# compbio-UofT/shrimp

Measured on AMD Instinct MI355X. Metric: reads/sec mapped (whole node), 100bp LS reads vs 3Gbp ref, 1/2/4/8 GPUs, higher is better.
Workload: dtype int16

## Files before the change

include/gmapper_hip.h:

```cpp
#ifndef GMAPPER_HIP_H
#define GMAPPER_HIP_H

#include <stddef.h>
#include <stdint.h>
#include <stdbool.h>

#ifdef __cplusplus
extern "C" {
#endif

#define GM_OK            0
#define GM_E_NODEVICE   -1
#define GM_E_ARG        -2
#define GM_E_NOTSETUP   -3
#define GM_E_RANGE      -4
#define GM_E_OVERFLOW   -5
#define GM_E_NOMEM      -6

const char *gm_last_error(void);
int gm_abi_sizeof(int which);
int gm_device_count(void);

typedef struct gm_params {
  int match_score, mismatch_score;
// ... 233 lines not shown
  int half_paired;
  int match_mode;
} gm_pair_opts_t;
void gm_pair_opts_default(gm_pair_opts_t *o);
int gm_map_pairs(gm_session_t *s, int n_pairs, int len1, const uint32_t *mates1_packed, int len2, const uint32_t *mates2_packed,
                 const char *names1, const char *names2, const gm_pair_opts_t *opts,
                 char **sam, size_t *sam_len, gm_map_stats_t *stats);
int gm_map_pairs_cs(gm_session_t *s, int n_pairs, int len1, const uint32_t *mates1_packed, const uint8_t *initbp1, int len2, const uint32_t *mates2_packed,
                    const uint8_t *initbp2, const char *names1, const char *names2, const gm_pair_opts_t *opts,
                    char **sam, size_t *sam_len, gm_map_stats_t *stats);
int gm_map_pairs_file(gm_session_t *s, const char *path1, const char *path2, int fastq, int qual_delta, const gm_pair_opts_t *opts,
                      char **sam, size_t *sam_len, gm_map_stats_t *stats);
int gm_map_pairs_file_cb(gm_session_t *s, const char *path1, const char *path2, int fastq, int qual_delta, const gm_pair_opts_t *opts, size_t chunk_pairs,
                         gm_write_fn write, void *ctx, gm_map_stats_t *stats);
int gm_map_pairs_cs_fastq(gm_session_t *s, int n_pairs, int len1, const uint32_t *mates1_packed, const uint8_t *initbp1, int len2, const uint32_t *mates2_packed,
                          const uint8_t *initbp2, const char *names1, const char *names2, const char *quals1, const char *quals2, int qual_delta,
                          const gm_pair_opts_t *opts, char **sam, size_t *sam_len, gm_map_stats_t *stats);
int gm_map_pairs_fastq(gm_session_t *s, int n_pairs, int len1, const uint32_t *mates1_packed, int len2, const uint32_t *mates2_packed,
                       const char *names1, const char *names2, const char *quals1, const char *quals2, int qual_delta,
                       const gm_pair_opts_t *opts, char **sam, size_t *sam_len, gm_map_stats_t *stats);

#define GM_MERGE_OUT_SAM              0
#define GM_MERGE_OUT_UNALIGNED_READS  1
#define GM_MERGE_OUT_ALIGNED_READS    2
typedef struct gm_merge_options {
  int max_outputs;
  int max_alignments;
  int strata;
  int half_paired;
  int sam_unaligned;
  int single_best;
  int all_contigs;
  int no_mapping_qualities;
  int leave_mapq;
  int no_improper_mappings;
  int min_mapq;
  int fastq;
  int threads;
  int output;
  int header_given;
  const char *command_line;
} gm_merge_options_t;
void gm_merge_options_default(gm_merge_options_t *o);
int gm_merge_sam(const gm_merge_options_t *opts, const char *reads_text, size_t reads_len, int n_files, const char *const *sam_text,
                 const size_t *sam_len, char **out, size_t *out_len);

int gm_debug_tophits(gm_session_t *s, int n_reads, int read_len, const uint32_t *reads_packed,
                     long long *rows, long cap, long *n_rows);
int gm_debug_tophits_cs(gm_session_t *s, int n_reads, int n_colours, const uint32_t *colours_packed, const uint8_t *initbp,
                        long long *rows, long cap, long *n_rows);

int gm_last_lookup_timing(gm_session_t *s, double *ms, uint64_t *alg_bytes, int *launches);
const char *gm_last_lookup_kernel(void);

#ifdef __cplusplus
}
#endif
#endif
```

shrimp_amd/csrc/gm_anchors.hip:

```cpp
#include <cstring>
#include <algorithm>
#include "gm_common.h"
#include "gm_internal.h"
#include <rocprim/device/device_segmented_radix_sort.hpp>

template <bool BIG> struct K2Idx { typedef uint16_t type; static constexpr uint32_t none = 0xFFFFu; };
template <> struct K2Idx<true> { typedef uint32_t type; static constexpr uint32_t none = 0xFFFFFFFFu; };

template <bool BIG>
struct K2Ws {
  typedef typename K2Idx<BIG>::type idx_t;
  uint64_t* key;
  uint32_t* aux;
  idx_t* nxt;
  idx_t* ord;
  idx_t* first;
  uint32_t* hk;
  uint16_t* hr;
  int16_t*  cache;
};

#ifdef K2_STAMPS
__device__ unsigned long long k2_stamps[8];
#define K2_STAMP(i) do { if (lane == 0) { const unsigned long long t_ = __builtin_amdgcn_s_memtime(); atomicAdd(&k2_stamps[i], t_ - t_prev); t_prev = t_; } } while (0)
extern "C" int gm_debug_k2_stamps(unsigned long long* out) {
  unsigned long long z[8] = {0, 0, 0, 0, 0, 0, 0, 0};
  if (hipMemcpyFromSymbol(out, HIP_SYMBOL(k2_stamps), sizeof z) != hipSuccess) return GM_E_NODEVICE;
  if (hipMemcpyToSymbol(HIP_SYMBOL(k2_stamps), z, sizeof z) != hipSuccess) return GM_E_NODEVICE;
  return GM_OK;
}
#else
#define K2_STAMP(i) do { } while (0)
#endif
template <bool BIG> __device__ __forceinline__ void k2_sync() { if (BIG) __threadfence(); __syncthreads(); }

template <bool BIG, typename T> __device__ void k2_bitonic(T* key, int npad, int lane) {
  for (int k = 2; k <= npad; k <<= 1)
    for (int j = k >> 1; j > 0; j >>= 1) {
      for (int t = lane; t < (npad >> 1); t += GM_WAVE) {
        const int i = ((t & ~(j - 1)) << 1) | (t & (j - 1));
        const int l = i | j;
        const bool up = ((i & k) == 0);
        const T a = key[i], b = key[l];
        if ((a > b) == up) { key[i] = b; key[l] = a; }
      }
      k2_sync<BIG>();
    }
}

template <typename T> __device__ __forceinline__ T k2_xor_lane(T v, int dl) { return (T)__shfl_xor(v, dl); }
template <> __device__ __forceinline__ uint64_t k2_xor_lane<uint64_t>(uint64_t v, int dl) {
  const uint32_t lo = (uint32_t)__shfl_xor((int)(uint32_t)v, dl), hi = (uint32_t)__shfl_xor((int)(uint32_t)(v >> 32), dl);
  return ((uint64_t)hi << 32) | lo;
}
template <typename T, int R> __device__ __forceinline__ void k2_bitonic_regs(T* key, int lane) {
  T v[R];
#pragma unroll
  for (int j = 0; j < R; j++) v[j] = key[lane * R + j];
#pragma unroll
  for (int k = 2; k <= 64 * R; k <<= 1) {
#pragma unroll
    for (int d = k >> 1; d > 0; d >>= 1) {
      if (d < R) {
#pragma unroll
        for (int j = 0; j < R; j++) if ((j & d) == 0) {
          const bool up = (((lane * R + j) & k) == 0);
          const T a = v[j], b = v[j | d];
          const bool sw = (a > b) == up;
          v[j] = sw ? b : a; v[j | d] = sw ? a : b;
        }
      } else {
        const int dl = d / R;
        const bool lower = (lane & dl) == 0;
#pragma unroll
        for (int j = 0; j < R; j++) {
          const bool up = (((lane * R + j) & k) == 0);
          const T o = k2_xor_lane<T>(v[j], dl);
          const bool less = v[j] < o;
          v[j] = ((up == lower) == less) ? v[j] : o;
        }
      }
    }
  }
#pragma unroll
  for (int j = 0; j < R; j++) key[lane * R + j] = v[j];
}
template <bool BIG, typename T, int RMAX = 16> __device__ void k2_sort(T* key, int npad, int lane) {
  if (!BIG && npad <= 64 * RMAX) {
    if (npad == 64) k2_bitonic_regs<T, 1>(key, lane); else if (npad == 128) k2_bitonic_regs<T, 2>(key, lane);
    else if (npad == 256) k2_bitonic_regs<T, 4>(key, lane); else if (npad == 512) k2_bitonic_regs<T, 8>(key, lane);
    else if (npad == 1024 || RMAX < 32) k2_bitonic_regs<T, 16>(key, lane);
    else k2_bitonic_regs<T, RMAX>(key, lane);
    __syncthreads();
  } else k2_bitonic<BIG, T>(key, npad, lane);
}

struct K2Box { long long x, y; int length, width; };
__device__ __forceinline__ K2Box k2_join2(long long x0, long long y0, int l0, int w0, long long x1, long long y1, int l1, int w1) {
  long long nw0 = x0 + y0, sw0 = x0 - y0, ne0 = sw0 + 2 * (w0 - 1), se0 = nw0 + 2 * (l0 - 1);
  long long nw1 = x1 + y1, sw1 = x1 - y1, ne1 = sw1 + 2 * (w1 - 1), se1 = nw1 + 2 * (l1 - 1);
  long long nw_min = min(nw0, nw1), sw_min = min(sw0, sw1), ne_max = max(ne0, ne1), se_max = max(se0, se1);
  K2Box r;
  if ((nw_min + sw_min) % 2 != 0) nw_min--;
  r.x = (nw_min + sw_min) / 2;
  r.y = nw_min - r.x;
  if ((ne_max - sw_min) % 2 != 0) ne_max++;
  r.width = (int)((ne_max - sw_min) / 2 + 1);
  if ((se_max - nw_min) % 2 != 0) se_max++;
  r.length = (int)((se_max - nw_min) / 2 + 1);
  return r;
}

__device__ __forceinline__ int k2_threshold(double frac, int absval, int base) {
  return frac < 0 ? absval : (int)((double)base * frac);
}

template <bool BIG>
__device__ void k2_exact_order(K2Ws<BIG>& ws, int n, int NL, int max_n_kmers) {
  typedef typename K2Idx<BIG>::type idx_t;
  const idx_t NONE = (idx_t)K2Idx<BIG>::none;
  for (int o = 0; o < NL; o++) ws.first[o] = NONE;
  for (int t = n - 1; t >= 0; t--) {
    const uint64_t k = ws.key[t];
    const int off = (int)(k & 0xFFFF) * max_n_kmers + (int)((k >> 16) & 0xFFFF);
    ws.nxt[t] = ws.first[off]; ws.first[off] = (idx_t)t;
  }
  int load = 0;
  auto pos_of = [&](int t) -> uint32_t { return (uint32_t)(ws.key[t] >> 32); };
  auto down = [&](int node) {
    for (;;) {
      int left = node * 2, right = left + 1, mn = node;
      if (left <= load && ws.hk[left - 1] < ws.hk[node - 1]) mn = left;
      if (right <= load && ws.hk[right - 1] < ws.hk[mn - 1]) mn = right;
      if (mn == node) break;
      uint32_t tk = ws.hk[mn - 1]; ws.hk[mn - 1] = ws.hk[node - 1]; ws.hk[node - 1] = tk;
      uint16_t tr = ws.hr[mn - 1]; ws.hr[mn - 1] = ws.hr[node - 1]; ws.hr[node - 1] = tr;
      node = mn;
    }
  };
  for (int o = 0; o < NL; o++) {
    if (ws.first[o] == NONE) continue;
    ws.hk[load] = pos_of((int)ws.first[o]); ws.hr[load] = (uint16_t)o; load++;
    int node = load, parent = node / 2;
    while (node > 1 && ws.hk[node - 1] < ws.hk[parent - 1]) {
      uint32_t tk = ws.hk[parent - 1]; ws.hk[parent - 1] = ws.hk[node - 1]; ws.hk[node - 1] = tk;
      uint16_t tr = ws.hr[parent - 1]; ws.hr[parent - 1] = ws.hr[node - 1]; ws.hr[node - 1] = tr;
      node = parent; parent = node / 2;
// ... 74 lines not shown
    if (valid) {
      c = ck[r]; t = (int)(c & 0xFFFF);
      const uint64_t k = ws.key[t]; const uint32_t au = ws.aux[t];
      x = (long long)(k >> 32); y = (int)(au & 0x7FFF); cn = (int)(au >> 16); span = ix.seed[(int)(k & 0xFFFF)].span;
    }
    uint32_t cp = (uint32_t)__shfl_up((int)c, 1); if (lane == 0) cp = carry_c;
    if (valid) {
      head = true;
      if (r > 0 && (cp >> 16) == (c >> 16)) {
        const int tp = (int)(cp & 0xFFFF);
        const long long xp = (long long)(ws.key[tp] >> 32); const uint32_t aup = ws.aux[tp];
        head = !((int)(aup >> 16) == cn && (xp - (long long)(aup & 0x7FFF)) == (x - y));
      }
    }
    carry_c = (uint32_t)__shfl((int)c, GM_WAVE - 1);
    int hidx = (valid && head) ? r : -1;
    for (int d = 1; d < GM_WAVE; d <<= 1) { const int o = __shfl_up(hidx, d); if (lane >= d) hidx = max(hidx, o); }
    hidx = max(hidx, carry_head);
    carry_head = __shfl(hidx, GM_WAVE - 1);
    k2_sync<false>();
    if (valid && head) { ck[r] = ((uint32_t)span << 16) | (uint32_t)t; ((uint32_t*)&ws.key[t])[0] = 1u; }
    k2_sync<false>();
    if (valid && !head) {
      const int th = (int)(ck[hidx] & 0xFFFF);
      const long long xh = (long long)(ws.key[th] >> 32);
      atomicMax(&ck[hidx], ((uint32_t)(x + span - xh) << 16) | (uint32_t)th);
      atomicAdd(&((uint32_t*)&ws.key[th])[0], 1u);
      atomicOr(&ws.aux[t], 0x8000u);
    }
  }
  k2_sync<false>();
  for (int r = lane; r < n; r += GM_WAVE) {
    const uint32_t c = ck[r]; const int t = (int)(c & 0xFFFF);
    if (ws.aux[t] & 0x8000u) continue;
    const uint64_t k = ws.key[t];
    ws.key[t] = (k & 0xFFFFFFFF00000000ull) | ((uint64_t)(c >> 16) << 16) | (uint64_t)min((uint32_t)k, 0xFFFFu);
  }
  k2_sync<false>();
  int na = 0;
  for (int c0 = 0; c0 < n; c0 += GM_WAVE) {
    const int t = c0 + lane;
    uint64_t k = 0; uint32_t au = 0x8000u;
    if (t < n) { k = ws.key[t]; au = ws.aux[t]; }
    const bool alive = !(au & 0x8000u);
    const unsigned long long bal = __ballot(alive);
    k2_sync<false>();
    if (alive) { const int d = na + __popcll(bal & ((1ull << lane) - 1ull)); ws.key[d] = k; ws.aux[d] = au; }
    na += __popcll(bal);
    k2_sync<false>();
  }
  return na;
}

template <bool BIG, bool DETECT>
__device__ int k2_windows(const GmIndexDev& ix, const GmScoreDev& sc, K2Ws<BIG>& ws, int na, int read_len, int window_len,
                          GmHit* H, uint32_t* hitx, int hcap, int lane, bool* sensitive, int rs) {
  const int match = sc.match;
  const uint32_t mp_n = sc.match_mode == 3 ? ix.mp.cnt[rs ^ 1] : 0u;
  const uint32_t* mp_row = sc.match_mode == 3 ? ix.mp.rows + (size_t)(rs ^ 1) * GM_MP_CAP : nullptr;
  const int mp_dmin = ix.mp.dmin[rs & 1], mp_dmax = ix.mp.dmax[rs & 1];
  int nh = 0; bool sens = false;
  for (int c0 = 0; c0 < na; c0 += GM_WAVE) {
    const int i = c0 + lane;
    bool pass = false; GmHit h; uint32_t myx = 0;
    if (i < na) {
      const uint64_t ai = ws.key[i]; const uint32_t aui = ws.aux[i];
      const long long xi = (long long)(ai >> 32); const int yi = (int)(aui & 0x7FFF);
      const int leni = (int)((ai >> 16) & 0xFFFF), wi = (int)(ai & 0xFFFF);
      const int cn = (int)(aui >> 16);
      myx = (uint32_t)xi;
      const long long coff = ix.contig_off[cn];
      const long long clen = (long long)ix.contig_off[cn + 1] - coff;
      int w_len = window_len;
      if ((long long)w_len > clen) w_len = (int)clen;
      long long gend = (xi - coff) + read_len - 1 - yi;
      if (gend > clen - 1) gend = clen - 1;
      const long long gstart = (gend >= window_len) ? gend - window_len : 0;
      int max_idx = i;
      int max_score = leni * match;
      bool heavy_mp = false;
      if (sc.match_mode == 3 && mp_n <= (uint32_t)GM_MP_CAP) {
        const uint32_t reg = (uint32_t)xi >> ix.region_bits;
        heavy_mp = gm_mp_reach(mp_row, mp_n, (long long)reg + mp_dmin, (long long)reg + mp_dmax);
        if (!heavy_mp && reg > 0 && ((uint32_t)xi & ((1u << ix.region_bits) - 1u)) < (uint32_t)ix.region_overlap)
          heavy_mp = gm_mp_reach(mp_row, mp_n, (long long)reg - 1 + mp_dmin, (long long)reg - 1 + mp_dmax);
      }
      if (!sc.gapless && (sc.match_mode == 2 || (sc.match_mode == 3 && !heavy_mp)) && wi == 1) max_score = -1;
      bool tie_sibling = false;
      for (int j = i - 1; !sc.gapless && j >= 0; j--) {
        const uint64_t aj = ws.key[j];
        const long long xj = (long long)(aj >> 32);
        if (xj < coff + gstart) break;
        const int yj = (int)(ws.aux[j] & 0x7FFF);
        if (yj >= yi) continue;
        int short_len, long_len;
        if (xi - yi > xj - yj) { short_len = (yi - yj) + leni; long_len = (int)(xi - xj) + leni; }
        else { short_len = (int)(xi - xj) + leni; long_len = (yi - yj) + leni; }
        int tmp;
        if (long_len > short_len) tmp = short_len * match - sc.b_go - (long_len - short_len) * sc.b_ge;
        else tmp = short_len * match;
        if (tmp > max_score) { max_idx = j; max_score = tmp; tie_sibling = false; }
        else if (DETECT && tmp == max_score && max_idx != i && xj == (long long)(ws.key[max_idx] >> 32)) tie_sibling = true;
      }
      const int base = (read_len < w_len ? read_len : w_len) * match;
      if (sc.gapless || sc.match_mode == 1 || (sc.match_mode == 3 && heavy_mp) || max_score >= k2_threshold(sc.wgen_thr_frac, sc.wgen_abs, base)) {
        const uint64_t am = ws.key[max_idx]; const uint32_t aum = ws.aux[max_idx];
        const long long xm = (long long)(am >> 32);
        if (DETECT && max_idx != i && (tie_sibling || xm == xi)) sens = true;
        const int x_len = (int)(xi - xm) + leni;
        long long goff;
        if ((window_len - x_len) / 2 < xm - coff) goff = (xm - coff) - (window_len - x_len) / 2; else goff = 0;
        if (goff + w_len > clen) goff = clen - w_len;
        K2Box b;
        if (max_idx < i) {
          b = k2_join2(xi - coff - goff, yi, leni, 1, xm - coff - goff, (int)(aum & 0x7FFF), (int)((am >> 16) & 0xFFFF), 1);
        } else { b.x = xi - coff - goff; b.y = yi; b.length = leni; b.width = 1; }
        h.g_off = (uint32_t)goff; h.ax = (int32_t)b.x; h.ay = (int32_t)b.y; h.alen = b.length; h.awidth = b.width;
        h.score_window_gen = max_score; h.score_vector = -1; h.pct_score_vector = 0;
        h.cn = (uint16_t)cn; h.w_len = (uint16_t)w_len;
        const int mt = (max_idx == i) ? wi : wi + (int)(am & 0xFFFF);
        h.matches = (uint16_t)min(mt, 0xFFFF); h.flags = 0;
        pass = true;
      }
    }
    const unsigned long long bal = __ballot(pass);
    if (pass) {
      const int slot = nh + __popcll(bal & ((1ull << lane) - 1ull));
      if (slot < hcap) { H[slot] = h; if (DETECT) hitx[slot] = myx; }
    }
    nh += __popcll(bal);
  }
  if (DETECT) *sensitive = __any(sens);
  return nh;
}

template <bool BIG, int RMAX = 16>
__global__ void __launch_bounds__(GM_WAVE)
k_anchors(GmIndexDev ix, GmScoreDev sc, int n_reads, int read_len, int window_len, int max_n_kmers, int NL,
          const uint64_t* __restrict__ surv, const uint32_t* __restrict__ surv_cnt, int scap,
          int n_heavy, const uint32_t* __restrict__ heavy_list, const uint64_t* __restrict__ seg_off, const uint32_t* __restrict__ seg_n,
          uint64_t* __restrict__ big_keys, uint32_t* __restrict__ big_aux, uint32_t* __restrict__ big_nxt, uint32_t* __restrict__ big_ord,
          GmHit* __restrict__ hits, uint16_t* __restrict__ perm, uint32_t* __restrict__ hit_cnt, int hcap,
          unsigned long long* __restrict__ stats,
          int lcap, int lmin) {
  typedef typename K2Idx<BIG>::type idx_t;
  extern __shared__ __align__(16) uint8_t smem_raw[];
  __shared__ int sh_na;
  const int lane = threadIdx.x;
#ifdef K2_STAMPS
  unsigned long long t_prev = __builtin_amdgcn_s_memtime();
#endif
  int rs, n;
  K2Ws<BIG> ws;
  uint8_t* base = smem_raw;
  if (BIG) {
    if ((int)blockIdx.x >= n_heavy) return;
    rs = (int)heavy_list[blockIdx.x];
    if ((sc.skip_strands >> (rs & 1)) & 1) { if (lane == 0) hit_cnt[rs] = 0; return; }
    n = (int)seg_n[blockIdx.x];
    const uint64_t o = seg_off[blockIdx.x];
    ws.key = big_keys + o; ws.aux = big_aux + o; ws.nxt = (idx_t*)(big_nxt + o); ws.ord = (idx_t*)(big_ord + o);
  } else {
    rs = blockIdx.x;
    const uint32_t n_all = ((sc.skip_strands >> (rs & 1)) & 1) ? 0u : surv_cnt[rs];
    if (n_all == 0 || n_all > (uint32_t)scap) { if (lane == 0 && lmin == 0) hit_cnt[rs] = 0; return; }
    if (n_all <= (uint32_t)lmin || n_all > (uint32_t)lcap) return;
    n = (int)n_all;
    ws.key = (uint64_t*)base;                    base += (size_t)lcap * 8;
    ws.aux = (uint32_t*)base;                    base += (size_t)lcap * 4;
    ws.nxt = (idx_t*)base;                       base += (size_t)lcap * sizeof(idx_t);
    ws.ord = (idx_t*)base;                       base += (size_t)lcap * sizeof(idx_t);
  }
  ws.hk = (uint32_t*)base;                       base += (size_t)NL * 4;
  ws.first = (idx_t*)base;                       base += (size_t)((NL + 1) & ~1) * sizeof(idx_t);
  ws.hr = (uint16_t*)base;                       base += (size_t)((NL + 1) & ~1) * 2;
  ws.cache = (int16_t*)base;
  uint32_t* scratch32 = (uint32_t*)ws.nxt;
  GmHit* H = hits + (size_t)rs * hcap;
  int npad = 64; while (npad < n) npad <<= 1;

  auto load_sorted = [&]() {
    if (!BIG) {
      const uint64_t* sv = surv + (size_t)rs * scap;
      for (int t = lane; t < npad; t += GM_WAVE) ws.key[t] = (t < n) ? sv[t] : ~0ull;
      k2_sync<BIG>();
      k2_sort<BIG, uint64_t, RMAX>(ws.key, npad, lane);
    }
    K2_STAMP(0);
    if (!BIG && ix.n_contigs <= GM_WAVE) {
      const uint32_t my_off = lane < ix.n_contigs ? ix.contig_off[lane] : 0xFFFFFFFFu;
      for (int t0 = 0; t0 < n; t0 += GM_WAVE) {
        const int t = t0 + lane;
        const uint64_t k = t < n ? ws.key[t] : 0ull;
        const uint32_t x = (uint32_t)(k >> 32);
        int lo = 0, hi = ix.n_contigs;
        for (int it = 0; it < 6; it++) {
          const int m = (lo + hi) >> 1;
          const uint32_t v = (uint32_t)__shfl((int)my_off, m);
          const bool open = hi - lo > 1, le = v <= x;
          lo = (open && le) ? m : lo; hi = (open && !le) ? m : hi;
        }
        if (t < n) ws.aux[t] = (uint32_t)((k >> 16) & 0x7FFF) | ((uint32_t)lo << 16);
      }
    } else
    for (int t = lane; t < n; t += GM_WAVE) {
      const uint64_t k = ws.key[t];
      const uint32_t x = (uint32_t)(k >> 32);
      int lo = 0, hi = ix.n_contigs;
      while (hi - lo > 1) { int m = (lo + hi) >> 1; if (ix.contig_off[m] <= x) lo = m; else hi = m; }
      ws.aux[t] = (uint32_t)((k >> 16) & 0x7FFF) | ((uint32_t)lo << 16);
    }
    k2_sync<BIG>();
  };

  auto sort_windows = [&](int nhc, bool detect) -> bool {
    bool sens = false;
    uint16_t* P = perm + (size_t)rs * hcap;
    if (nhc > 0) {
      int hp = 64; while (hp < nhc) hp <<= 1;
      for (int t = lane; t < hp; t += GM_WAVE) {
        uint64_t k = ~0ull;
        if (t < nhc) {
          const uint32_t go = __hip_atomic_load(&H[t].g_off, __ATOMIC_RELAXED, __HIP_MEMORY_SCOPE_AGENT);
          const uint32_t cw = __hip_atomic_load((const uint32_t*)&H[t].cn, __ATOMIC_RELAXED, __HIP_MEMORY_SCOPE_AGENT);
          k = ((uint64_t)(cw & 0xFFFF) << 48) | ((uint64_t)go << 16) | (uint64_t)t;
        }
        ws.key[t] = k;
      }
      k2_sync<BIG>();
      k2_sort<BIG, uint64_t, RMAX>(ws.key, hp, lane);
      for (int t = lane; t < nhc; t += GM_WAVE) {
        P[t] = (uint16_t)(ws.key[t] & 0xFFFF);
        if (detect && t > 0 && (ws.key[t] >> 16) == (ws.key[t - 1] >> 16) &&
            scratch32[ws.key[t] & 0xFFFF] == scratch32[ws.key[t - 1] & 0xFFFF]) sens = true;
      }
    }
    return __any(sens);
  };

  int na = 0, nh = 0;
  bool need_exact = BIG;
  load_sorted();
  K2_STAMP(1);
  if (!BIG) {
    na = k2_collapse_par<RMAX>(ix, *(K2Ws<false>*)&ws, scratch32, n, npad, read_len, lane);
    K2_STAMP(2);
    bool sens = false;
    nh = k2_windows<BIG, true>(ix, sc, ws, na, read_len, window_len, H, scratch32, hcap, lane, &sens, rs);
    k2_sync<BIG>();
    K2_STAMP(3);
    need_exact = sens;
    if (!need_exact) need_exact = sort_windows(min(nh, hcap), true);
    K2_STAMP(4);
  }
  if (need_exact) {
    if (!BIG) { k2_sync<BIG>(); load_sorted(); }
    bool danger = false;
    for (int t = lane + 1; t < n; t += GM_WAVE) {
      const uint64_t a = ws.key[t - 1], b = ws.key[t];
      danger |= ((a >> 32) == (b >> 32)) && (((a >> 16) & 0xFFFF) != ((b >> 16) & 0xFFFF));
    }
    danger = __any(danger);
    for (int d = lane; d < read_len; d += GM_WAVE) ws.cache[d] = -1;
    k2_sync<BIG>();
    if (lane == 0) {
      GS_ADD(stats, GS_EXACT_ORDER, 1ull);
      if (danger) k2_exact_order<BIG>(ws, n, NL, max_n_kmers);
      sh_na = k2_collapse_seq<BIG>(ix, ws, n, read_len);
    }
    k2_sync<BIG>();
    na = sh_na;
    bool dummy;
    nh = k2_windows<BIG, false>(ix, sc, ws, na, read_len, window_len, H, scratch32, hcap, lane, &dummy, rs);
    k2_sync<BIG>();
    sort_windows(min(nh, hcap), false);
  }
  if (lane == 0) {
    hit_cnt[rs] = (uint32_t)nh;
    GS_ADD(stats, GS_ANCHORS, na);
    GS_ADD(stats, GS_WINDOWS, min(nh, hcap));
    if (nh > hcap) GS_ADD(stats, GS_OVERFLOW_HITS, 1ull);
  }
}

static size_t k2_lds_bytes(bool big, int scap, int NL, int read_len) {
  size_t b = (size_t)NL * 4 + (size_t)((NL + 1) & ~1) * (big ? 4 : 2) + (size_t)((NL + 1) & ~1) * 2 + (size_t)read_len * 2;
  if (!big) b += (size_t)scap * (8 + 4 + 2 + 2);
  return (b + 15) & ~(size_t)15;
}

int gm_launch_anchors(const GmIndexDev& ix, const GmScoreDev& sc, int n_reads, int read_len, int window_len,
                      const uint64_t* d_surv, const uint32_t* d_surv_cnt, int scap,
                      GmHit* d_hits, uint16_t* d_perm, uint32_t* d_hit_cnt, int hcap, unsigned long long* d_stats, hipStream_t stream) {
  const int max_n_kmers = std::max(0, read_len - ix.min_seed_span + 1);
  const int NL = ix.n_seeds * max_n_kmers;
  if (n_reads == 0) return GM_OK;
  const bool split = scap >= 2048 && !(gm_tune("GM_K2_WIDE") && atoi(gm_tune("GM_K2_WIDE")) == 0);
  const size_t lds = k2_lds_bytes(false, scap, NL, read_len), lds_a = k2_lds_bytes(false, split ? 1024 : scap, NL, read_len);
  if (lds > 64 * 1024) {
    if (lds > 160 * 1024) { gm_set_error("anchor kernel LDS %zu too large", lds); return GM_E_ARG; }
    GM_HIP(gm_lds_at_least((const void*)k_anchors<false>, lds)); GM_HIP(gm_lds_at_least((const void*)k_anchors<false, 32>, lds));
  }
  hipLaunchKernelGGL(k_anchors<false>, dim3(n_reads * 2), dim3(GM_WAVE), lds_a, stream, ix, sc, n_reads, read_len, window_len, max_n_kmers, NL,
                     d_surv, d_surv_cnt, scap, 0, (const uint32_t*)nullptr, (const uint64_t*)nullptr, (const uint32_t*)nullptr,
                     (uint64_t*)nullptr, (uint32_t*)nullptr, (uint32_t*)nullptr, (uint32_t*)nullptr,
                     d_hits, d_perm, d_hit_cnt, hcap, d_stats, split ? 1024 : scap, 0);
  if (split)
  hipLaunchKernelGGL((k_anchors<false, 32>), dim3(n_reads * 2), dim3(GM_WAVE), lds, stream, ix, sc, n_reads, read_len, window_len, max_n_kmers, NL,
                     d_surv, d_surv_cnt, scap, 0, (const uint32_t*)nullptr, (const uint64_t*)nullptr, (const uint32_t*)nullptr,
                     (uint64_t*)nullptr, (uint32_t*)nullptr, (uint32_t*)nullptr, (uint32_t*)nullptr,
                     d_hits, d_perm, d_hit_cnt, hcap, d_stats, scap, 1024);
  GM_HIP(hipGetLastError());
  return GM_OK;
}

int gm_launch_anchors_heavy(const GmIndexDev& ix, const GmScoreDev& sc, int n_reads, int read_len, int window_len,
                            int n_heavy, const uint32_t* d_heavy_list, const uint64_t* d_seg_off, const uint32_t* d_seg_n,
                            const uint32_t* d_seg_begin32, const uint32_t* d_seg_end32, uint64_t total_keys,
                            uint64_t* d_keys_in, uint64_t* d_keys_sorted, uint32_t* d_aux, uint32_t* d_nxt, uint32_t* d_ord,
                            GmHit* d_hits, uint16_t* d_perm, uint32_t* d_hit_cnt, int hcap, unsigned long long* d_stats, hipStream_t stream) {
  if (n_heavy == 0) return GM_OK;
  const int max_n_kmers = std::max(0, read_len - ix.min_seed_span + 1);
  const int NL = ix.n_seeds * max_n_kmers;
  size_t tmp_bytes = 0; void* tmp = nullptr;
  hipError_t e = rocprim::segmented_radix_sort_keys(nullptr, tmp_bytes, d_keys_in, d_keys_sorted, (unsigned int)total_keys, (unsigned int)n_heavy,
                                                    d_seg_begin32, d_seg_end32, 0, 64, stream);
  if (e != hipSuccess) { gm_set_error("segmented_radix_sort_keys size query: %s", hipGetErrorString(e)); return GM_E_NODEVICE; }
  GM_HIP(hipMalloc(&tmp, tmp_bytes ? tmp_bytes : 16));
  e = rocprim::segmented_radix_sort_keys(tmp, tmp_bytes, d_keys_in, d_keys_sorted, (unsigned int)total_keys, (unsigned int)n_heavy,
                                         d_seg_begin32, d_seg_end32, 0, 64, stream);
  if (e != hipSuccess) { (void)hipFree(tmp); gm_set_error("segmented_radix_sort_keys: %s", hipGetErrorString(e)); return GM_E_NODEVICE; }
  const size_t lds = k2_lds_bytes(true, 0, NL, read_len);
  hipLaunchKernelGGL(k_anchors<true>, dim3(n_heavy), dim3(GM_WAVE), lds, stream, ix, sc, n_reads, read_len, window_len, max_n_kmers, NL,
                     (const uint64_t*)nullptr, (const uint32_t*)nullptr, 0, n_heavy, d_heavy_list, d_seg_off, d_seg_n,
                     d_keys_sorted, d_aux, d_nxt, d_ord, d_hits, d_perm, d_hit_cnt, hcap, d_stats, 0, 0);
  GM_HIP(hipGetLastError());
  GM_HIP(hipStreamSynchronize(stream));
  (void)hipFree(tmp);
  return GM_OK;
}
```

shrimp_amd/gmapper.py:

```python
from __future__ import annotations

import ctypes as C
import os
import numpy as np

_HERE = os.path.dirname(os.path.abspath(__file__))
LIB_PATH = os.environ.get("GM_LIB_PATH") or os.path.join(_HERE, "libgmapper_hip.so")


class GmError(RuntimeError):
    pass


class Params(C.Structure):
    _fields_ = [("match_score", C.c_int), ("mismatch_score", C.c_int),
                ("a_gap_open_score", C.c_int), ("a_gap_extend_score", C.c_int),
                ("b_gap_open_score", C.c_int), ("b_gap_extend_score", C.c_int),
                ("window_len", C.c_double), ("window_overlap", C.c_double), ("window_gen_threshold", C.c_double),
                ("sw_vect_threshold", C.c_double), ("sw_full_threshold", C.c_double),
                ("match_mode", C.c_int), ("num_outputs", C.c_int), ("num_tmp_outputs", C.c_int), ("anchor_width", C.c_int),
                ("region_bits", C.c_int), ("region_overlap", C.c_int), ("list_cutoff", C.c_uint32),
                ("hash_filter_calls", C.c_int), ("tiebreak_rev", C.c_int), ("sam_unaligned", C.c_int), ("longest_read_len", C.c_int),
                ("strata", C.c_int), ("max_alignments", C.c_int),
                ("colour_space", C.c_int), ("crossover_score", C.c_int), ("indel_taboo_len", C.c_int), ("pr_xover", C.c_double),
# ... 46 lines not shown
        setattr(o, k, int(v))
    o.output = MERGE_OUT[output] if isinstance(output, str) else int(output)
    if command_line is not None:
        o.command_line = command_line if isinstance(command_line, bytes) else command_line.encode()
    texts = [bytes(t) for t in sam_texts]
    arr = (C.c_char_p * len(texts))(*texts); lens = (C.c_size_t * len(texts))(*[len(t) for t in texts])
    out = C.c_void_p(); ol = C.c_size_t()
    _check(L.gm_merge_sam(C.byref(o), reads_text, len(reads_text), len(texts), arr, lens, C.byref(out), C.byref(ol)), "gm_merge_sam")
    res = C.string_at(out, ol.value) if out.value else b""
    if out.value: L.gm_free(out)
    return res


class Anchor(C.Structure):
    _fields_ = [("x", C.c_longlong), ("y", C.c_longlong), ("length", C.c_int), ("width", C.c_int),
                ("weight", C.c_int), ("cn", C.c_int), ("score", C.c_int)]


class SwFullResults(C.Structure):
    _fields_ = [(n, C.c_int) for n in ("read_start", "rmapped", "genome_start", "gmapped", "matches", "mismatches",
                                       "insertions", "deletions", "score", "posterior_score", "pct_posterior_score")] + \
               [("dbalign", C.c_void_p), ("qralign", C.c_void_p), ("qual", C.c_void_p), ("posterior", C.c_double), ("mqv", C.c_int)] + \
               [(n, C.c_double) for n in ("z0", "z1", "z2", "z3", "pr_top_random_at_location", "pr_missed_mp", "insert_size_denom")] + \
               [("crossovers", C.c_int), ("dup", C.c_bool), ("in_use", C.c_bool)]


class SwFullRec(C.Structure):
    _fields_ = [(n, C.c_int) for n in ("score", "read_start", "rmapped", "gmapped", "matches", "mismatches", "insertions", "deletions", "crossovers", "status")] + \
               [("genome_start", C.c_int64), ("ops_off", C.c_uint64), ("n_ops", C.c_uint32)]


class PostRec(C.Structure):
    _fields_ = [("posterior", C.c_double), ("matches", C.c_int), ("mismatches", C.c_int), ("crossovers", C.c_int), ("status", C.c_int), ("by_host", C.c_int),
                ("qual_len", C.c_uint32), ("qual_off", C.c_uint64)]


SW_FULL_REC_DTYPE = np.dtype(SwFullRec)
POST_REC_DTYPE = np.dtype(PostRec)
ANCHOR_DTYPE = np.dtype(Anchor)


EXPORTS = ["gm_map_pairs_file", "gm_map_reads_file_cb", "gm_map_pairs_file_cb", "gm_preprocess_read_text", "gm_map_pairs_cs_fastq", "gm_map_reads_file", "gm_merge_options_default", "gm_merge_sam", "gm_release_cache", "gm_map_pairs_cs", "gm_last_error", "gm_device_count", "gm_params_default", "gm_params_default_cs", "gm_index_build", "gm_index_build_fasta", "gm_index_n_contigs", "gm_index_contig", "gm_sam_header", "gm_index_build_timing", "gm_index_free", "gm_index_list_cutoff",
           "gm_index_save", "gm_index_load", "gm_index_bytes", "gm_index_n_slabs", "gm_index_has_buckets", "gm_index_get_list", "gm_index_device_array", "gm_index_meta", "gm_index_alloc_like",
           "sw_vector_setup", "sw_vector", "sw_vector_stats", "sw_vector_cleanup", "gm_sw_vector_batch", "gm_sw_vector_batch_bounded",
           "sw_gapless_setup", "sw_gapless", "sw_gapless_stats", "gm_sw_gapless_batch",
           "sw_full_ls_setup", "sw_full_ls", "sw_full_ls_cleanup", "sw_full_ls_stats",
           "sw_full_cs_setup", "sw_full_cs", "sw_full_cs_cleanup", "sw_full_cs_stats", "gm_sw_vector_batch_cs",
           "gm_sw_full_ls_batch", "gm_sw_full_cs_batch", "gm_sw_full_batch_strings",
           "post_sw_setup", "post_sw", "post_sw_cleanup", "post_sw_stats", "gm_post_sw_batch", "gm_post_sw_batch_last_plan",
           "gm_index_genome_is_rna", "gm_index_get_windows", "gm_sw_vector_batch_ix", "gm_sw_vector_batch_bounded_ix", "gm_sw_gapless_batch_ix", "gm_sw_full_ls_batch_ix", "gm_sw_full_cs_batch_ix",
           "gm_post_sw_batch_ix", "gm_sw_full_batch_text", "gm_sw_full_batch_text_ix",
           "gm_session_create", "gm_session_free", "gm_sequence_to_bitfield", "gm_map_reads_text", "gm_map_reads", "gm_map_reads_fastq", "gm_map_reads_cs", "gm_map_reads_cs_fastq", "gm_map_reads_device", "gm_free", "gm_debug_tophits", "gm_debug_tophits_cs",
           "gm_pair_opts_default", "gm_map_pairs", "gm_map_pairs_fastq",
           "gm_last_lookup_timing", "gm_last_lookup_kernel", "gm_abi_sizeof"]

_lib = None


def lib():
    global _lib
    if _lib is not None:
        return _lib
    if not os.path.exists(LIB_PATH):
        raise GmError(f"{LIB_PATH} is missing: build it with `make -C shrimp_amd/csrc` (or __graft_entry__.build())")
    L = C.CDLL(LIB_PATH)
    u32p, vp = C.POINTER(C.c_uint32), C.c_void_p
    L.gm_last_error.restype = C.c_char_p
    L.gm_last_lookup_kernel.restype = C.c_char_p
    L.gm_device_count.restype = C.c_int
    L.gm_params_default.argtypes = [C.POINTER(Params)]
    L.gm_params_default_cs.argtypes = [C.POINTER(Params)]
    L.gm_index_build.argtypes = [C.POINTER(vp), C.c_int, C.c_int, C.POINTER(u32p), u32p, C.POINTER(C.c_char_p), C.c_int, C.POINTER(C.c_char_p), C.POINTER(Params)]
    L.gm_index_build_fasta.argtypes = [C.POINTER(vp), C.c_int, C.c_int, C.POINTER(C.c_char_p), C.c_int, C.POINTER(C.c_char_p), C.POINTER(Params)]
    L.gm_index_n_contigs.argtypes = [vp]; L.gm_index_n_contigs.restype = C.c_int
    L.gm_index_contig.argtypes = [vp, C.c_int, C.POINTER(C.c_char_p), u32p]
    L.gm_sam_header.argtypes = [vp, C.c_char_p, C.c_char_p, C.c_char_p, C.POINTER(vp), C.POINTER(C.c_size_t)]
    L.gm_index_build_timing.argtypes = [vp, C.POINTER(C.c_double), C.POINTER(C.c_double)]
    L.gm_index_free.argtypes = [vp]
    L.gm_index_save.argtypes = [vp, C.c_char_p]
    L.gm_index_load.argtypes = [C.POINTER(vp), C.c_int, C.c_char_p, C.POINTER(Params)]
    L.gm_index_list_cutoff.argtypes = [vp]; L.gm_index_list_cutoff.restype = C.c_uint32
    L.gm_index_bytes.argtypes = [vp]; L.gm_index_bytes.restype = C.c_uint64
    L.gm_index_n_slabs.argtypes = [vp]; L.gm_index_n_slabs.restype = C.c_int
    L.gm_index_has_buckets.argtypes = [vp]; L.gm_index_has_buckets.restype = C.c_int
    L.gm_index_get_list.argtypes = [vp, C.c_int, C.c_uint32, u32p, u32p, C.c_uint32]
    L.gm_index_device_array.argtypes = [vp, C.c_int, C.POINTER(vp), C.POINTER(C.c_uint64)]
    L.gm_index_meta.argtypes = [vp, vp, C.POINTER(C.c_uint64)]
    L.gm_index_alloc_like.argtypes = [C.POINTER(vp), C.c_int, vp, C.c_uint64]
    L.sw_vector_setup.argtypes = [C.c_int] * 9 + [C.c_bool]
    L.sw_vector.argtypes = [u32p, C.c_int, C.c_int, u32p, C.c_int, u32p, C.c_int, C.c_bool]
    L.gm_sw_vector_batch.argtypes = [C.c_int, u32p, C.c_uint64, C.POINTER(C.c_int64), C.POINTER(C.c_int), u32p, C.c_int, C.POINTER(C.c_int), C.POINTER(C.c_int)]
    L.gm_sw_vector_batch_bounded.argtypes = [C.c_int, u32p, C.c_uint64, C.POINTER(C.c_int64), C.POINTER(C.c_int), u32p, C.c_int, C.POINTER(C.c_int), C.c_int, C.POINTER(C.c_int),
                                             C.POINTER(C.c_uint8)]
    L.sw_gapless_setup.argtypes = [C.c_int, C.c_int, C.c_bool]
    L.sw_gapless.argtypes = [u32p, C.c_int, u32p, C.c_int, C.c_int, C.c_int, u32p, C.c_int, C.c_bool]
    L.gm_sw_gapless_batch.argtypes = [C.c_int, u32p, u32p, C.c_uint64, C.POINTER(C.c_int64), C.POINTER(C.c_int), u32p, C.c_int, C.POINTER(C.c_int), C.POINTER(C.c_int),
                                      C.POINTER(C.c_int), C.POINTER(C.c_int), C.POINTER(C.c_int)]
    L.sw_full_ls_setup.argtypes = [C.c_int] * 8 + [C.c_bool, C.c_int]
    L.sw_full_ls.argtypes = [u32p, C.c_int, C.c_int, u32p, C.c_int, C.c_int, C.c_int, C.POINTER(SwFullResults), C.c_bool, C.POINTER(Anchor), C.c_int, C.c_int]
    L.sw_full_ls.restype = None
    L.sw_full_cs_setup.argtypes = [C.c_int] * 9 + [C.c_bool, C.c_int, C.c_int]
    L.sw_full_cs.argtypes = [u32p, C.c_int, C.c_int, u32p, C.c_int, C.c_int, C.c_int, C.POINTER(SwFullResults), C.c_bool, C.c_bool, C.POINTER(Anchor), C.c_int, C.c_int, vp]
    L.sw_full_cs.restype = None
    L.gm_sw_vector_batch_cs.argtypes = [C.c_int, u32p, u32p, C.c_uint64, C.POINTER(C.c_int64), C.POINTER(C.c_int), u32p, C.c_int, C.POINTER(C.c_int), C.POINTER(C.c_int), C.POINTER(C.c_int)]
    L.gm_sw_full_ls_batch.argtypes = [C.c_int, u32p, C.c_uint64, C.POINTER(C.c_int64), C.POINTER(C.c_int), u32p, C.c_int, C.POINTER(C.c_int), vp, vp, C.POINTER(C.c_int), vp,
                                      C.c_int, vp, C.POINTER(vp), C.POINTER(C.c_uint64)]
    L.gm_sw_full_cs_batch.argtypes = [C.c_int, u32p, C.c_uint64, C.POINTER(C.c_int64), C.POINTER(C.c_int), u32p, C.c_int, C.POINTER(C.c_int), vp, vp, vp, C.POINTER(C.c_int), vp,
                                      C.c_int, C.c_int, C.c_int, vp, C.POINTER(vp), C.POINTER(C.c_uint64)]
    L.gm_sw_full_batch_strings.argtypes = [C.c_int, vp, vp, C.c_uint64, u32p, C.c_uint64, u32p, C.c_int, C.c_int, C.c_int, C.POINTER(vp), C.POINTER(vp)]
    L.post_sw_setup.argtypes = [C.c_int] + [C.c_double] * 6 + [C.c_bool, C.c_bool, C.c_int, C.c_int, C.c_bool]
    L.post_sw.argtypes = [u32p, C.c_int, C.c_char_p, C.POINTER(SwFullResults)]; L.post_sw.restype = None
    L.gm_post_sw_batch.argtypes = [C.c_int, vp, vp, C.c_uint64, u32p, C.c_uint64, u32p, C.c_int, C.POINTER(C.c_int), vp, vp, C.c_int, vp, C.POINTER(vp), C.POINTER(vp),
                                   C.POINTER(C.c_uint64)]
    L.gm_post_sw_batch_last_plan.argtypes = [C.c_int, C.POINTER(C.c_int), C.POINTER(C.c_int), C.POINTER(C.c_int)]
    ipt, i64p, u8p = C.POINTER(C.c_int), C.POINTER(C.c_int64), C.POINTER(C.c_uint8)
    win = [vp, C.c_int, ipt, u8p, i64p, ipt]
    L.gm_index_genome_is_rna.argtypes = [vp]
    L.gm_index_get_windows.argtypes = win + [C.c_int, u32p, C.c_int]
    L.gm_sw_vector_batch_ix.argtypes = win + [u32p, C.c_int, ipt, ipt, C.c_int, ipt]
    L.gm_sw_vector_batch_bounded_ix.argtypes = win + [u32p, C.c_int, ipt, C.c_int, ipt, u8p]
    L.gm_sw_gapless_batch_ix.argtypes = [vp, C.c_int, ipt, u8p, C.c_int, u32p, C.c_int, ipt, ipt, ipt, ipt, C.c_int, ipt]
# ... 869 lines not shown
```

Baseline: 3.520 million.

## Collapse anchors by sorting on diagonal keys and reuse window keys for sorting

Replaces the old anchor pipeline (load a sorted list, then run a parallel collapse) with a single bitonic sort over packed diagonal keys read straight from the survivor buffer. Runs on each diagonal are merged with wave-level scans, sorted again by position, and tagged with contig numbers through a lane-resident binary search. Window emission now also writes sort keys in place, so the window sort can skip rebuilding them. The old path stays available under a tuning flag, and a new guard rejects reads of 32768 or longer or more than 16 seeds, since the packed key fields cannot hold them.

Result: no change. 3.550 million (median of 6 runs) (+0.8%).

```diff
diff --git a/include/gmapper_hip.h b/include/gmapper_hip.h
--- a/include/gmapper_hip.h
+++ b/include/gmapper_hip.h
@@ -309,6 +309,7 @@
 
 int gm_last_lookup_timing(gm_session_t *s, double *ms, uint64_t *alg_bytes, int *launches);
 const char *gm_last_lookup_kernel(void);
+const char *gm_last_anchor_path(void);
 
 #ifdef __cplusplus
 }
diff --git a/shrimp_amd/csrc/gm_anchors.hip b/shrimp_amd/csrc/gm_anchors.hip
--- a/shrimp_amd/csrc/gm_anchors.hip
+++ b/shrimp_amd/csrc/gm_anchors.hip
@@ -53,10 +53,10 @@
   const uint32_t lo = (uint32_t)__shfl_xor((int)(uint32_t)v, dl), hi = (uint32_t)__shfl_xor((int)(uint32_t)(v >> 32), dl);
   return ((uint64_t)hi << 32) | lo;
 }
-template <typename T, int R> __device__ __forceinline__ void k2_bitonic_regs(T* key, int lane) {
+template <typename T, int R, typename LD> __device__ __forceinline__ void k2_bitonic_regs(T* key, int lane, LD ld) {
   T v[R];
 #pragma unroll
-  for (int j = 0; j < R; j++) v[j] = key[lane * R + j];
+  for (int j = 0; j < R; j++) v[j] = ld(lane * R + j);
 #pragma unroll
   for (int k = 2; k <= 64 * R; k <<= 1) {
 #pragma unroll
@@ -85,6 +85,7 @@
 #pragma unroll
   for (int j = 0; j < R; j++) key[lane * R + j] = v[j];
 }
+template <typename T, int R> __device__ __forceinline__ void k2_bitonic_regs(T* key, int lane) { k2_bitonic_regs<T, R>(key, lane, [&](int i) -> T { return key[i]; }); }
 template <bool BIG, typename T, int RMAX = 16> __device__ void k2_sort(T* key, int npad, int lane) {
   if (!BIG && npad <= 64 * RMAX) {
     if (npad == 64) k2_bitonic_regs<T, 1>(key, lane); else if (npad == 128) k2_bitonic_regs<T, 2>(key, lane);
@@ -93,6 +94,20 @@
     else k2_bitonic_regs<T, RMAX>(key, lane);
     __syncthreads();
   } else k2_bitonic<BIG, T>(key, npad, lane);
+}
+
+template <typename T, int RMAX, typename LD> __device__ void k2_sort_ld(T* key, int npad, int lane, LD ld) {
+  if (npad <= 64 * RMAX) {
+    if (npad == 64) k2_bitonic_regs<T, 1>(key, lane, ld); else if (npad == 128) k2_bitonic_regs<T, 2>(key, lane, ld);
+    else if (npad == 256) k2_bitonic_regs<T, 4>(key, lane, ld); else if (npad == 512) k2_bitonic_regs<T, 8>(key, lane, ld);
+    else if (npad == 1024 || RMAX < 32) k2_bitonic_regs<T, 16>(key, lane, ld);
+    else k2_bitonic_regs<T, RMAX>(key, lane, ld);
+    __syncthreads();
+  } else {
+    for (int t0 = 0; t0 < npad; t0 += GM_WAVE) { const T k = ld(t0 + lane); __syncthreads(); key[t0 + lane] = k; }
+    __syncthreads();
+    k2_bitonic<false, T>(key, npad, lane);
+  }
 }
 
 struct K2Box { long long x, y; int length, width; };
@@ -273,9 +288,79 @@
   return na;
 }
 
+__device__ __forceinline__ int k2_contig_of(const GmIndexDev& ix, bool in_lanes, uint32_t my_off, uint32_t x) {
+  int lo = 0, hi = ix.n_contigs;
+  if (in_lanes) {
+    for (int it = 0; it < 6; it++) {
+      const int m = (lo + hi) >> 1;
+      const uint32_t v = (uint32_t)__shfl((int)my_off, m);
+      const bool open = hi - lo > 1, le = v <= x;
+      lo = (open && le) ? m : lo; hi = (open && !le) ? m : hi;
+    }
+  } else
+    while (hi - lo > 1) { const int m = (lo + hi) >> 1; if (ix.contig_off[m] <= x) lo = m; else hi = m; }
+  return lo;
+}
+
+__device__ int k2_diag_runs(const GmIndexDev& ix, K2Ws<false>& ws, uint32_t* pl, int n, int read_len, int lane) {
+  const bool in_lanes = ix.n_contigs <= GM_WAVE;
+  const uint32_t my_off = (in_lanes && lane < ix.n_contigs) ? ix.contig_off[lane] : 0xFFFFFFFFu;
+  int na = 0, c_hidx = 0; uint32_t c_e = 0, c_dlo = 0, c_w2 = 0xFFFFFFFFu, c_yh = 0;
+  for (int c0 = 0; c0 < n; c0 += GM_WAVE) {
+    const int r = c0 + lane; const bool valid = r < n;
+    const uint64_t dk = ws.key[r];
+    const uint32_t y = (uint32_t)(dk >> 4) & 0x7FFFu, dlo = (uint32_t)(dk >> 19), dhi = (uint32_t)(dk >> 51) & 1u;
+    const uint32_t x = dlo + y - (uint32_t)read_len;
+    const int cn = k2_contig_of(ix, in_lanes, my_off, valid ? x : 0u);
+    const uint32_t w2 = (uint32_t)cn | (dhi << 16);
+    uint32_t dlo_p = (uint32_t)__shfl_up((int)dlo, 1), w2_p = (uint32_t)__shfl_up((int)w2, 1);
+    if (lane == 0) { dlo_p = c_dlo; w2_p = c_w2; }
+    const bool head = valid && (dlo != dlo_p || w2 != w2_p);
+    const unsigned long long hb = __ballot(head);
+    const unsigned long long le = hb & (~0ull >> (63 - lane));
+    const int hl = le ? 63 - __clzll((long long)le) : -1;
+    const int hidx = hl >= 0 ? c0 + hl : c_hidx;
+    uint32_t yh = (uint32_t)__shfl((int)y, hl & 63); if (hl < 0) yh = c_yh;
+    uint32_t e = valid ? y + (uint32_t)ix.seed[(int)(dk & 0xF)].span : 0u;
+    if (hl < 0 && lane == 0) e = max(e, c_e);
+    uint32_t p = ((uint32_t)(hl + 1) << 16) | e;
+    for (int d = 1; d < GM_WAVE; d <<= 1) { const uint32_t o = (uint32_t)__shfl_up((int)p, d); if (lane >= d) p = max(p, o); }
+    const uint32_t emax = p & 0xFFFFu;
+    const bool last = valid && (lane == GM_WAVE - 1 || r == n - 1 || ((hb >> 1 >> lane) & 1ull));
+    if (last) {
+      const int a = na + __popcll(le) - 1;
+      const uint32_t xh = dlo + yh - (uint32_t)read_len;
+      ws.key[a] = ((uint64_t)xh << 32) | ((uint64_t)yh << 16) | (uint64_t)(uint32_t)a;
+      pl[a] = ((emax - yh) << 16) | min((uint32_t)(r - hidx + 1), 0xFFFFu);
+    }
+    na += __popcll(hb);
+    c_hidx = __shfl(hidx, GM_WAVE - 1); c_e = (uint32_t)__shfl((int)emax, GM_WAVE - 1); c_yh = (uint32_t)__shfl((int)yh, GM_WAVE - 1);
+    c_dlo = (uint32_t)__shfl((int)dlo, GM_WAVE - 1); c_w2 = (uint32_t)__shfl((int)w2, GM_WAVE - 1);
+  }
+  k2_sync<false>();
+  return na;
+}
+template <int RMAX>
+__device__ void k2_diag_heads(const GmIndexDev& ix, K2Ws<false>& ws, const uint32_t* pl, int na, int lane) {
+  int hp = 64; while (hp < na) hp <<= 1;
+  k2_sort_ld<uint64_t, (RMAX < 16 ? RMAX : 16)>(ws.key, hp, lane, [&](int t) -> uint64_t { return t < na ? ws.key[t] : ~0ull; });
+  const bool in_lanes = ix.n_contigs <= GM_WAVE;
+  const uint32_t my_off = (in_lanes && lane < ix.n_contigs) ? ix.contig_off[lane] : 0xFFFFFFFFu;
+  for (int c0 = 0; c0 < na; c0 += GM_WAVE) {
+    const int i = c0 + lane; const bool valid = i < na;
+    const uint64_t s = ws.key[i];
+    const int cn = k2_contig_of(ix, in_lanes, my_off, valid ? (uint32_t)(s >> 32) : 0u);
+    if (valid) {
+      ws.key[i] = (s & 0xFFFFFFFF00000000ull) | (uint64_t)pl[(int)(s & 0xFFFF)];
+      ws.aux[i] = ((uint32_t)(s >> 16) & 0x7FFFu) | ((uint32_t)cn << 16);
+    }
+  }
+  k2_sync<false>();
+}
+
 template <bool BIG, bool DETECT>
 __device__ int k2_windows(const GmIndexDev& ix, const GmScoreDev& sc, K2Ws<BIG>& ws, int na, int read_len, int window_len,
-                          GmHit* H, uint32_t* hitx, int hcap, int lane, bool* sensitive, int rs) {
+                          GmHit* H, uint32_t* hitx, int hcap, int lane, bool* sensitive, int rs, uint64_t* wkey = nullptr) {
   const int match = sc.match;
   const uint32_t mp_n = sc.match_mode == 3 ? ix.mp.cnt[rs ^ 1] : 0u;
   const uint32_t* mp_row = sc.match_mode == 3 ? ix.mp.rows + (size_t)(rs ^ 1) * GM_MP_CAP : nullptr;
@@ -347,7 +432,10 @@
     const unsigned long long bal = __ballot(pass);
     if (pass) {
       const int slot = nh + __popcll(bal & ((1ull << lane) - 1ull));
-      if (slot < hcap) { H[slot] = h; if (DETECT) hitx[slot] = myx; }
+      if (slot < hcap) {
+        H[slot] = h; if (DETECT) hitx[slot] = myx;
+        if (wkey) wkey[slot] = ((uint64_t)h.cn << 48) | ((uint64_t)h.g_off << 16) | (uint64_t)slot;
+      }
     }
     nh += __popcll(bal);
   }
@@ -363,7 +451,8 @@
           uint64_t* __restrict__ big_keys, uint32_t* __restrict__ big_aux, uint32_t* __restrict__ big_nxt, uint32_t* __restrict__ big_ord,
           GmHit* __restrict__ hits, uint16_t* __restrict__ perm, uint32_t* __restrict__ hit_cnt, int hcap,
           unsigned long long* __restrict__ stats,
-          int lcap, int lmin) {
+          int lcap, int lmin,
+          int two_sorts) {
   typedef typename K2Idx<BIG>::type idx_t;
   extern __shared__ __align__(16) uint8_t smem_raw[];
   __shared__ int sh_na;
@@ -434,11 +523,13 @@
     k2_sync<BIG>();
   };
 
-  auto sort_windows = [&](int nhc, bool detect) -> bool {
+  auto sort_windows = [&](int nhc, bool detect, const uint64_t* wsrc) -> bool {
     bool sens = false;
     uint16_t* P = perm + (size_t)rs * hcap;
     if (nhc > 0) {
       int hp = 64; while (hp < nhc) hp <<= 1;
+      if (!BIG && wsrc) k2_sort_ld<uint64_t, (RMAX < 16 ? RMAX : 16)>(ws.key, hp, lane, [&](int t) -> uint64_t { return t < nhc ? wsrc[t] : ~0ull; });
+      else {
       for (int t = lane; t < hp; t += GM_WAVE) {
         uint64_t k = ~0ull;
         if (t < nhc) {
@@ -450,6 +541,7 @@
       }
       k2_sync<BIG>();
       k2_sort<BIG, uint64_t, RMAX>(ws.key, hp, lane);
+      }
       for (int t = lane; t < nhc; t += GM_WAVE) {
         P[t] = (uint16_t)(ws.key[t] & 0xFFFF);
         if (detect && t > 0 && (ws.key[t] >> 16) == (ws.key[t - 1] >> 16) &&
@@ -461,17 +553,37 @@
 
   int na = 0, nh = 0;
   bool need_exact = BIG;
-  load_sorted();
-  K2_STAMP(1);
+#ifdef GM_TUNING
+  const bool two = two_sorts != 0;
+#else
+  constexpr bool two = false;
+#endif
+  if (BIG || two) { load_sorted(); K2_STAMP(1); }
   if (!BIG) {
-    na = k2_collapse_par<RMAX>(ix, *(K2Ws<false>*)&ws, scratch32, n, npad, read_len, lane);
+    uint64_t* wkey = nullptr;
+    if (two) na = k2_collapse_par<RMAX>(ix, *(K2Ws<false>*)&ws, scratch32, n, npad, read_len, lane);
+    else {
+      const uint64_t* sv = surv + (size_t)rs * scap;
+      const uint64_t L = (uint64_t)read_len;
+      k2_sort_ld<uint64_t, RMAX>(ws.key, npad, lane, [&](int t) -> uint64_t {
+        if (t >= n) return ~0ull;
+        const uint64_t k = sv[t], y = (k >> 16) & 0x7FFFull;
+        return (((k >> 32) + L - y) << 19) | (y << 4) | (k & 0xFull);
+      });
+      K2_STAMP(0);
+      na = k2_diag_runs(ix, *(K2Ws<false>*)&ws, scratch32, n, read_len, lane);
+      K2_STAMP(1);
+      k2_diag_heads<RMAX>(ix, *(K2Ws<false>*)&ws, scratch32, na, lane);
+      int hp = 64; while (hp < na) hp <<= 1;
+      if (na + hp <= lcap) wkey = ws.key + na;
+    }
     K2_STAMP(2);
     bool sens = false;
-    nh = k2_windows<BIG, true>(ix, sc, ws, na, read_len, window_len, H, scratch32, hcap, lane, &sens, rs);
+    nh = k2_windows<BIG, true>(ix, sc, ws, na, read_len, window_len, H, scratch32, hcap, lane, &sens, rs, wkey);
     k2_sync<BIG>();
     K2_STAMP(3);
     need_exact = sens;
-    if (!need_exact) need_exact = sort_windows(min(nh, hcap), true);
+    if (!need_exact) need_exact = sort_windows(min(nh, hcap), true, wkey);
     K2_STAMP(4);
   }
   if (need_exact) {
@@ -494,7 +606,7 @@
     bool dummy;
     nh = k2_windows<BIG, false>(ix, sc, ws, na, read_len, window_len, H, scratch32, hcap, lane, &dummy, rs);
     k2_sync<BIG>();
-    sort_windows(min(nh, hcap), false);
+    sort_windows(min(nh, hcap), false, nullptr);
   }
   if (lane == 0) {
     hit_cnt[rs] = (uint32_t)nh;
@@ -504,6 +616,8 @@
   }
 }
 
+static const char* g_k2_path = "";
+extern "C" const char* gm_last_anchor_path(void) { return g_k2_path; }
 static size_t k2_lds_bytes(bool big, int scap, int NL, int read_len) {
   size_t b = (size_t)NL * 4 + (size_t)((NL + 1) & ~1) * (big ? 4 : 2) + (size_t)((NL + 1) & ~1) * 2 + (size_t)read_len * 2;
   if (!big) b += (size_t)scap * (8 + 4 + 2 + 2);
@@ -516,6 +630,9 @@
   const int max_n_kmers = std::max(0, read_len - ix.min_seed_span + 1);
   const int NL = ix.n_seeds * max_n_kmers;
   if (n_reads == 0) return GM_OK;
+  if (read_len >= 32768 || ix.n_seeds > 16) { gm_set_error("anchor kernel: read length %d / %d seeds beyond the diagonal key's fields", read_len, ix.n_seeds); return GM_E_ARG; }
+  const int two_sorts = (gm_tune("GM_K2_TWO_SORTS") && atoi(gm_tune("GM_K2_TWO_SORTS")) != 0) ? 1 : 0;
+  g_k2_path = two_sorts ? "two_sorts" : "diagonal";
   const bool split = scap >= 2048 && !(gm_tune("GM_K2_WIDE") && atoi(gm_tune("GM_K2_WIDE")) == 0);
   const size_t lds = k2_lds_bytes(false, scap, NL, read_len), lds_a = k2_lds_bytes(false, split ? 1024 : scap, NL, read_len);
   if (lds > 64 * 1024) {
@@ -525,12 +642,12 @@
   hipLaunchKernelGGL(k_anchors<false>, dim3(n_reads * 2), dim3(GM_WAVE), lds_a, stream, ix, sc, n_reads, read_len, window_len, max_n_kmers, NL,
                      d_surv, d_surv_cnt, scap, 0, (const uint32_t*)nullptr, (const uint64_t*)nullptr, (const uint32_t*)nullptr,
                      (uint64_t*)nullptr, (uint32_t*)nullptr, (uint32_t*)nullptr, (uint32_t*)nullptr,
-                     d_hits, d_perm, d_hit_cnt, hcap, d_stats, split ? 1024 : scap, 0);
+                     d_hits, d_perm, d_hit_cnt, hcap, d_stats, split ? 1024 : scap, 0, two_sorts);
   if (split)
   hipLaunchKernelGGL((k_anchors<false, 32>), dim3(n_reads * 2), dim3(GM_WAVE), lds, stream, ix, sc, n_reads, read_len, window_len, max_n_kmers, NL,
                      d_surv, d_surv_cnt, scap, 0, (const uint32_t*)nullptr, (const uint64_t*)nullptr, (const uint32_t*)nullptr,
                      (uint64_t*)nullptr, (uint32_t*)nullptr, (uint32_t*)nullptr, (uint32_t*)nullptr,
-                     d_hits, d_perm, d_hit_cnt, hcap, d_stats, scap, 1024);
+                     d_hits, d_perm, d_hit_cnt, hcap, d_stats, scap, 1024, two_sorts);
   GM_HIP(hipGetLastError());
   return GM_OK;
 }
@@ -554,7 +671,7 @@
   const size_t lds = k2_lds_bytes(true, 0, NL, read_len);
   hipLaunchKernelGGL(k_anchors<true>, dim3(n_heavy), dim3(GM_WAVE), lds, stream, ix, sc, n_reads, read_len, window_len, max_n_kmers, NL,
                      (const uint64_t*)nullptr, (const uint32_t*)nullptr, 0, n_heavy, d_heavy_list, d_seg_off, d_seg_n,
-                     d_keys_sorted, d_aux, d_nxt, d_ord, d_hits, d_perm, d_hit_cnt, hcap, d_stats, 0, 0);
+                     d_keys_sorted, d_aux, d_nxt, d_ord, d_hits, d_perm, d_hit_cnt, hcap, d_stats, 0, 0, 0);
   GM_HIP(hipGetLastError());
   GM_HIP(hipStreamSynchronize(stream));
   (void)hipFree(tmp);
diff --git a/shrimp_amd/gmapper.py b/shrimp_amd/gmapper.py
--- a/shrimp_amd/gmapper.py
+++ b/shrimp_amd/gmapper.py
@@ -122,7 +122,7 @@
            "gm_post_sw_batch_ix", "gm_sw_full_batch_text", "gm_sw_full_batch_text_ix",
            "gm_session_create", "gm_session_free", "gm_sequence_to_bitfield", "gm_map_reads_text", "gm_map_reads", "gm_map_reads_fastq", "gm_map_reads_cs", "gm_map_reads_cs_fastq", "gm_map_reads_device", "gm_free", "gm_debug_tophits", "gm_debug_tophits_cs",
            "gm_pair_opts_default", "gm_map_pairs", "gm_map_pairs_fastq",
-           "gm_last_lookup_timing", "gm_last_lookup_kernel", "gm_abi_sizeof"]
+           "gm_last_lookup_timing", "gm_last_lookup_kernel", "gm_last_anchor_path", "gm_abi_sizeof"]
 
 _lib = None
 
@@ -137,6 +137,7 @@
     u32p, vp = C.POINTER(C.c_uint32), C.c_void_p
     L.gm_last_error.restype = C.c_char_p
     L.gm_last_lookup_kernel.restype = C.c_char_p
+    L.gm_last_anchor_path.restype = C.c_char_p
     L.gm_device_count.restype = C.c_int
     L.gm_params_default.argtypes = [C.POINTER(Params)]
     L.gm_params_default_cs.argtypes = [C.POINTER(Params)]
```
